# uzh-rpg/RVT

Hardware: AMD Instinct MI355X
Metric: event-tensors/sec (fwd+bwd) RVT-Base T=21 1Mpx; % MFMA roofline (higher is better)
Workload: dtype bf16; 1 GPU; RVT-Base, 1Mpx 20x360x640 (padded 384x640), T=21, B=24/GPU; global_batch=24, seq_len=21, parallelism=dp1, optimizer=AdamW(fused), hipgraph=off, upstream_grads=random cotangents on stage 2-4 features of all T frames

## Files before the change

### rvt_amd/csrc/capi_scan.hip

```cpp
#include "host.hpp"
#include "gemm.hpp"
#include "lstm_scan.hpp"
#include "lstm_scan2.hpp"
#include "lstm_scan3.hpp"

using namespace rvt;

extern "C" {
int rvt_lstm_scan_supported(int dtype, int C) {
    if (dtype != RVT_BF16 && dtype != RVT_F32) return 0;
    return C == 32 || C == 64 || C == 128;
}
}
template <class K> static int scan_grid(K kernel, int threads, int M, int tm) {
    const int resident_override = tuning().gemm_resident;
    const int n_tiles = (M + tm - 1) / tm;
    const int per_cu = resident_per_cu(kernel, threads, 1);
    return imax(1, imin(n_tiles, resident_override > 0 ? resident_override : 256 * per_cu));
}
template <class T, int C, int NW, int RB, bool W_LDS, bool W_REG = false>
static void launch_lstm_scan_fwd(const void* x_all, void* Hall, const float* c0, float* c_last, void* Csave, const void* W,
                                 const float* bias, void* gates_out, int M, int Tn, hipStream_t st) {
    constexpr int TM = (NW / (C / 32)) * RB * 32;
    auto k = lstm_scan_fwd_kernel<T, C, NW, RB, W_LDS, W_REG>;
// ... 89 lines not shown
            auto k = lstm_scan2_bwd_kernel;
            const int grid = scan_grid(k, 512, M, Scan2BwdSmem::TM);
            hipLaunchKernelGGL(k, dim3(grid), dim3(512), 0, st, (const bf16*)x_all, (const bf16*)Hall, (const bf16*)Csave, c0,
                               (const bf16*)dH, dc_last, (const bf16*)w, bias, (bf16*)dx_all, (bf16*)dh0, dc0, ws, M, T_steps);
            const size_t wn = (size_t)4 * C * 2 * C;
            FoldJobs fj;
            fj.add((const float*)ws, dw, grid, Scan2BwdSmem::REC, wn);
            fj.add((const float*)(ws + wn), db, grid, Scan2BwdSmem::REC, (size_t)4 * C);
            launch_fold_jobs(fj, st);
        }
        else if (C == 64) RVT_SCAN_BWD(bf16, 64, 4, true, false);
        else RVT_SCAN_BWD(bf16, 128, 4, false, false);
    } else {
        if (C == 32) RVT_SCAN_BWD(float, 32, 4, false, false);
        else if (C == 64) RVT_SCAN_BWD(float, 64, 4, false, false);
        else RVT_SCAN_BWD(float, 128, 4, false, false);
    }
#undef RVT_SCAN_BWD
    return check_launch("lstm_scan_bwd");
}


int rvt_lstm_scan3_rb(int C) { return (C == 256 ? tuning().lstm_scan3_rb256 : tuning().lstm_scan3_rb128) == 2 ? 2 : 1; }
int rvt_lstm_scan3_supported(int dtype, int C) {
    return dtype == RVT_BF16 && ((C == 256 && (tuning().lstm_scan3 & 1)) || (C == 128 && (tuning().lstm_scan3 & 2)));
}
int rvt_lstm_scan3_rows(int C, int M, int rb) {
    const int tm = 32 * (rb == 2 ? 2 : 1);
    return (M + tm - 1) / tm * tm;
}
int rvt_lstm_scan3_pack(const void* w, void* wp_fwd, void* wtp_bwd, int C, void* stream) {
    RVT_CHECK(C % 64 == 0 && w != nullptr, "lstm_scan3_pack: C=%d must be a multiple of 64", C);
    hipStream_t st = (hipStream_t)stream;
    const int pieces = (C / 64) * (2 * C / 16) * 8 * 64;
    const int grid = imax(1, imin(1024, (pieces + 255) / 256));
    if (wp_fwd != nullptr) hipLaunchKernelGGL(lstm_scan3_pack_kernel<false>, dim3(grid), dim3(256), 0, st, (const bf16*)w, (bf16*)wp_fwd, C);
    if (wtp_bwd != nullptr) hipLaunchKernelGGL(lstm_scan3_pack_kernel<true>, dim3(grid), dim3(256), 0, st, (const bf16*)w, (bf16*)wtp_bwd, C);
    return check_launch("lstm_scan3_pack");
}
int rvt_lstm_scan3_fwd(const void* x_all, void* Hall, const float* c0, float* c_last, void* Csave, const void* wp, const float* bias,
                       void* gsave, int dtype, int M, int C, int T_steps, int rb, void* stream) {
    RVT_CHECK(rvt_lstm_scan3_supported(dtype, C) && (rb == 1 || rb == 2), "lstm_scan3_fwd: not built for dtype=%d C=%d rb=%d", dtype, C, rb);
    RVT_CHECK(M >= 1 && T_steps >= 1 && (Csave == nullptr) == (gsave == nullptr), "lstm_scan3_fwd: empty problem, or only one of Csave / gsave");
    hipStream_t st = (hipStream_t)stream;
#define RVT_SCAN3_FWD(CC, RBB) do { auto k = lstm_scan3_fwd_kernel<CC, RBB>;                                                     \
        hipLaunchKernelGGL(k, dim3(scan_grid(k, CC, M, 32 * RBB)), dim3(CC), 0, st, (const bf16*)x_all, (bf16*)Hall, c0, c_last, \
                           (bf16*)Csave, (const bf16*)wp, bias, (bf16*)gsave, M, T_steps); } while (0)
    if (C == 256) { if (rb == 2) RVT_SCAN3_FWD(256, 2); else RVT_SCAN3_FWD(256, 1); }
    else { if (rb == 2) RVT_SCAN3_FWD(128, 2); else RVT_SCAN3_FWD(128, 1); }
#undef RVT_SCAN3_FWD
    return check_launch("lstm_scan3_fwd");
}
int rvt_lstm_scan3_bwd(const void* gsave, const void* Csave, const float* c0, const void* dH, const float* dc_last, const void* wtp,
                       void* dx_all, void* dz_all, void* dh0, float* dc0, int dtype, int M, int C, int T_steps, int rb, void* stream) {
    RVT_CHECK(rvt_lstm_scan3_supported(dtype, C) && (rb == 1 || rb == 2), "lstm_scan3_bwd: not built for dtype=%d C=%d rb=%d", dtype, C, rb);
    RVT_CHECK(M >= 1 && T_steps >= 1 && gsave != nullptr && Csave != nullptr && dx_all != nullptr && dz_all != nullptr,
              "lstm_scan3_bwd: empty problem / missing buffers");
    hipStream_t st = (hipStream_t)stream;
#define RVT_SCAN3_BWD(CC) do { auto k = lstm_scan3_bwd_kernel<CC>;                                                                       \
        hipLaunchKernelGGL(k, dim3(scan_grid(k, CC, M, 32)), dim3(CC), 0, st, (const bf16*)gsave, (const bf16*)Csave, c0, (const bf16*)dH, \
                           dc_last, (const bf16*)wtp, (bf16*)dx_all, (bf16*)dz_all, (bf16*)dh0, dc0, M, T_steps, rb); } while (0)
    if (C == 256) RVT_SCAN3_BWD(256); else RVT_SCAN3_BWD(128);
#undef RVT_SCAN3_BWD
    return check_launch("lstm_scan3_bwd");
}

}
```

### rvt_amd/csrc/capi_stage.hip

```cpp
#include <vector>
#include "host.hpp"

using namespace rvt;

namespace rvt {
int stage_blocks_fwd(const RvtStageDesc& d, const RvtStageRoutes& r, const void* inp, void* prepack, void* y0, void* x0,
                     const RvtBlockSaved* blk, int T, int B, void* stream) {
    const int C = d.C, F = T * B, dt = d.dtype;
    const int H = conv_out(d.H_in, d.k, d.stride, d.pad), W = conv_out(d.W_in, d.k, d.stride, d.pad), M = F * H * W;
    if (d.inp_u8 && rvt_stem_supported(dt, 1, d.Cin, C, d.k, d.stride, d.pad, d.w_raw)) {
        RVT_TRY(rvt_stem_fwd(inp, d.conv_w, d.ln_w, d.ln_b, y0, x0, dt, F, d.Cin, d.cin_pad, d.h_raw, d.w_raw, d.H_in, d.W_in, d.eps, stream));
    } else {
        if (d.inp_u8) {
            RVT_CHECK(prepack != nullptr, "stage forward: uint8 planes need the stem kernels (the host prepacks otherwise)");
            RVT_TRY(rvt_prepack_input(inp, 1, prepack, dt, F, d.Cin, d.h_raw, d.w_raw, d.H_in, d.W_in, d.cin_pad, stream));
            inp = prepack;
        }
        RVT_TRY(rvt_conv_fwd(inp, d.conv_w, y0, dt, F, d.H_in, d.W_in, d.cin_pad, C, d.k, d.stride, d.pad, stream));
        RVT_TRY(rvt_layernorm_fwd(y0, d.ln_w, d.ln_b, x0, dt, M, C, d.eps, stream));
    }
    const void* x = x0;
    for (int bi = 0; bi < 2 * d.num_blocks; bi++) {
        const RvtBlockWeights& bw = d.blocks[bi];
        const RvtBlockSaved& b = blk[bi];
// ... 54 lines not shown
}
}

extern "C" {

int rvt_stage_routes(const RvtStageDesc* dp, int T, int B, int save, int has_dws, int has_token_mask, RvtStageRoutes* out) {
    RVT_CHECK(dp != nullptr && out != nullptr && dp->struct_bytes == (int)sizeof(RvtStageDesc) && T >= 1 && B >= 1,
              "stage_routes: bad arguments (struct_bytes must be sizeof(RvtStageDesc) = %d)", (int)sizeof(RvtStageDesc));
    const RvtStageDesc& d = *dp;
    const RvtTuning& tn = tuning();
    const int dt = d.dtype, C = d.C, n_tok = d.ph * d.pw;
    const int Ms = B * conv_out(d.H_in, d.k, d.stride, d.pad) * conv_out(d.W_in, d.k, d.stride, d.pad);
    RvtStageRoutes r;
    memset(&r, 0, sizeof(r));

    r.attn_block = !(save && n_tok > 64) && tn.route_attn_block != 0 && rvt_attn_block_supported(dt, C, d.dim_head, n_tok);
    r.ln_linear = !r.attn_block && rvt_ln_linear_supported(dt, C, 3 * C);
    r.dgrad_ln_qkv = rvt_linear_dgrad_ln_supported(dt, C, 3 * C) != 0;
    r.dgrad_ln_fc1 = rvt_linear_dgrad_ln_supported(dt, C, 4 * C) != 0;
    r.attn_preln = (r.attn_block || r.dgrad_ln_qkv) && tn.route_attn_preln != 0 && !has_token_mask && d.num_blocks > 0 &&
                   d.blocks != nullptr && d.blocks[0].n1_w == nullptr;

    const int mlp_mode = tn.route_fused_mlp;
    const bool mlp_fused = mlp_mode != 0 && rvt_mlp_fused_supported(dt, C);
    if (mlp_mode != 0 && tn.route_mlp_bwd_fused != 0 && rvt_mlp_bwd_fused_supported(dt, C)) r.mlp_route = 1;
    else if (mlp_fused && (mlp_mode == 1 || C == 64 || C == 128)) r.mlp_route = save ? 2 : 1;
    r.mlp_bwd_both = r.mlp_route == 1 && rvt_mlp_bwd_both_supported(dt, C);
    r.mlp_bwd_dgrad = r.mlp_route == 2 && (mlp_mode == 1 || C == 64);
    r.mlp_store_pre = r.mlp_route == 2 && tn.route_mlp_store_pre != 0 && !r.mlp_bwd_dgrad;

    const int scan_mode = tn.route_lstm_scan;
    if (!has_dws && rvt_lstm_scan3_supported(dt, C) && !(C == 128 && Ms < 16384 && scan_mode != 0) && (save || T > 1)) {
        r.lstm_route = 3;
        r.lstm_scan3_rb = rvt_lstm_scan3_rb(C);
    } else if (!has_dws && scan_mode != 0 && rvt_lstm_scan_supported(dt, C) && !(scan_mode == -1 && T == 1 && !save) &&
               (scan_mode == 1 || C <= 64 || rvt_lstm_scan_saves_gates(dt, C))) {
        r.lstm_route = rvt_lstm_scan_saves_gates(dt, C) ? 2 : 1;
    }
    r.lstm_scan_wgrad = r.lstm_route == 1 && tn.route_lstm_scan_wgrad != 0 && rvt_lstm_scan_bwd_ws_floats(dt, C, Ms) > 0;
    r.conv_dgrad4 = tn.route_conv_dgrad4 != 0 && rvt_conv_dgrad4_supported(dt, d.H_in, d.W_in, d.Cin, C, d.k, d.stride, d.pad, T * B);
    r.driver_covers = !has_dws && !has_token_mask && (!save || r.mlp_route != 2);
    *out = r;
    return 0;
}

size_t rvt_stage_seq_fwd_ws_bytes(const RvtStageDesc* d, int T, int B) {
    RvtStageRoutes r;
    if (rvt_stage_routes(d, T, B, 0, 0, 0, &r) != 0) return 0;
    return stage_ws_bytes(*d, r, T, B);
}

int rvt_stage_seq_fwd(const RvtStageDesc* dp, const void* inp, const void* h0, const float* c0, void* Hall, float* c_last,
                      void* ws, size_t ws_bytes, int T, int B, void* stream) {
    RvtStageRoutes r;
    RVT_TRY(rvt_stage_routes(dp, T, B, 0, 0, 0, &r));
    const RvtStageDesc& d = *dp;
    RVT_CHECK(d.num_blocks >= 0 && d.blocks != nullptr && inp != nullptr && Hall != nullptr && c_last != nullptr, "stage_seq_fwd: bad arguments");
    RVT_CHECK((h0 == nullptr) == (c0 == nullptr), "stage_seq_fwd: h0 and c0 go together");
    RVT_CHECK(ws != nullptr && ws_bytes >= stage_ws_bytes(d, r, T, B), "stage_seq_fwd: workspace of %zu bytes < rvt_stage_seq_fwd_ws_bytes = %zu",
              ws_bytes, stage_ws_bytes(d, r, T, B));
    const int C = d.C, F = T * B, dt = d.dtype;
    const int H = conv_out(d.H_in, d.k, d.stride, d.pad), W = conv_out(d.W_in, d.k, d.stride, d.pad);
    RVT_CHECK(H % d.ph == 0 && W % d.pw == 0, "stage_seq_fwd: %dx%d not divisible by the partition %dx%d", H, W, d.ph, d.pw);
    const size_t e = elt_bytes(dt), tok = (size_t)F * H * W, act = tok * C * e;
    RVT_CHECK(tok * 4 * C < ((size_t)1 << 31), "stage_seq_fwd: %zu token rows exceed the operators' 32-bit sizes", tok);
    Carver cv{(char*)ws, ws_bytes, 256};
    void* bufs[3] = {cv.take(act), cv.take(act), cv.take(act)};
// ... 53 lines not shown
```

### rvt_amd/csrc/lstm_scan3.hpp

```cpp
#pragma once
#include "common.hpp"
#include "mlp.hpp"
#include "ppgemm.hpp"

namespace rvt {

template <int C, int RB> struct Scan3Geom {
    static constexpr int NW = C / 64, NT = 64 * NW, TM = 32 * RB;
    static constexpr int KT = C / 64;
    static constexpr int TILE = KT * TM * 128;
    static constexpr int NKF = 2 * C / 16;
    static constexpr int NKB = 4 * C / 16;
    static constexpr int PD = RB == 1 ? 4 : 8;
    static constexpr int WGS = RB == 1 ? 512 / C : 1;
    static_assert(C % 64 == 0 && NKF % PD == 0 && NKB % PD == 0, "geometry");
};

__device__ __forceinline__ bf16x8 scan3_as_frag(const u32x4& v) { return __builtin_bit_cast(bf16x8, v); }

template <int C, int RB> __device__ __forceinline__ void scan3_dma_tile(char* smem, int tile_off, const bf16* src, int rows, int wave, int lane) {
    typedef Scan3Geom<C, RB> G;
    const pp_rsrc rs = pp_make_rsrc(src, src != nullptr ? (unsigned)(rows * C * 2) : 0u);
    constexpr int NI = G::KT * (G::TM / 8), PER = NI / G::NW;
    static_assert(NI % G::NW == 0, "DMA pieces per wave");
#pragma unroll
    for (int q = 0; q < PER; q++) {
        const int u = wave * PER + q;
        const int kt = u / (G::TM / 8), rg = u % (G::TM / 8);
        const int r = 8 * rg + (lane >> 3);
        const int c = (lane & 7) ^ ((r >> 1) & 7) ^ ((r >> 4) & 7);
        pp_glds16(rs, smem, tile_off + kt * G::TM * 128 + rg * 1024, r * C * 2 + kt * 128 + c * 16, 0);
    }
}

template <int C, int RB>
__global__ void __launch_bounds__(C, (Scan3Geom<C, RB>::WGS * C) / 256)
lstm_scan3_fwd_kernel(const bf16* __restrict__ x_all, bf16* __restrict__ Hall, const float* __restrict__ c0, float* __restrict__ c_last,
                      bf16* __restrict__ Csave, const bf16* __restrict__ Wp, const float* __restrict__ bias, bf16* __restrict__ gsave,
                      int M, int Tn) {
    typedef bf16 T;
    typedef Scan3Geom<C, RB> G;
    constexpr int NW = G::NW, NT = G::NT, TM = G::TM, TILE = G::TILE, NKF = G::NKF, PD = G::PD;
    __shared__ __attribute__((aligned(1024))) char smem[4 * TILE];
    constexpr int OFF_X = 0, OFF_H = 2 * TILE;

    const int tid = threadIdx.x, lane = tid & 63, wave = wave_uniform(tid >> 6);
    const int li = lane & 31, half = lane >> 5;
    const size_t MC = (size_t)M * C;
    int ch[2];
    float nbf[2], nbi[2], nbo[2], tbg[2];
    int off0[RB][2];
#pragma unroll
    for (int cb = 0; cb < 2; cb++) {
        ch[cb] = 64 * wave + 32 * cb + li;
        nbf[cb] = bias[ch[cb]] * -1.4426950408889634f;
        nbi[cb] = bias[C + ch[cb]] * -1.4426950408889634f;
        nbo[cb] = bias[2 * C + ch[cb]] * -1.4426950408889634f;
        tbg[cb] = bias[3 * C + ch[cb]] * 2.8853900817779268f;
#pragma unroll
        for (int i = 0; i < RB; i++)
            off0[i][cb] = (int)(reinterpret_cast<char*>(opm_elem_ptr<T>(smem, TM, i * 32 + 4 * half, ch[cb])) - smem);
    }
    const pp_rsrc rw = pp_make_rsrc(Wp + (size_t)wave * NKF * 8 * 512, (unsigned)(NKF * 8 * 1024));
    const int lane16 = lane * 16;
    u32x4 bq[PD][4];
    auto issue = [&](u32x4 (&slot)[4], int p) {
#pragma unroll
        for (int j = 0; j < 4; j++) slot[j] = pp_load16(rw, ((p * 4 + j) << 10) + lane16);
    };
#pragma unroll
    for (int j = 0; j < PD; j++) issue(bq[j], j);

    const int n_tiles = (M + TM - 1) / TM;
    const size_t ntb = (size_t)n_tiles * RB;
    for (int tile = blockIdx.x; tile < n_tiles; tile += gridDim.x) {
        const int m0 = tile * TM;
        const int rows = M - m0 < TM ? M - m0 : TM;
        float creg[RB][2][16];
        lds_barrier();
        scan3_dma_tile<C, RB>(smem, OFF_H, Hall + (size_t)m0 * C, rows, wave, lane);
        scan3_dma_tile<C, RB>(smem, OFF_X, x_all + (size_t)m0 * C, rows, wave, lane);
#pragma unroll
        for (int i = 0; i < RB; i++)
#pragma unroll
            for (int cb = 0; cb < 2; cb++)
#pragma unroll
                for (int r = 0; r < 16; r++) {
                    const int row = m0 + i * 32 + acc_row(r, lane);
                    creg[i][cb][r] = (c0 != nullptr && row < M) ? c0[(size_t)row * C + ch[cb]] : 0.f;
                }
        pp_wait_vm<0>();
        lds_barrier();
        for (int t = 0; t < Tn; t++) {
            const int cur = t & 1;
            const char* const Ax = smem + OFF_X + cur * TILE;
            const char* const Ah = smem + OFF_H + cur * TILE;
            char* const An = smem + OFF_H + (cur ^ 1) * TILE;
            if (t + 1 < Tn) scan3_dma_tile<C, RB>(smem, OFF_X + (cur ^ 1) * TILE, x_all + (size_t)(t + 1) * MC + (size_t)m0 * C, rows, wave, lane);
#pragma unroll
            for (int cb = 0; cb < 2; cb++) {
                f32x16 acc[RB][4];
#pragma unroll
                for (int i = 0; i < RB; i++)
#pragma unroll
                    for (int g = 0; g < 4; g++) acc_zero(acc[i][g]);
#pragma unroll 1
                for (int k0 = 0; k0 < NKF; k0 += PD) {
#pragma unroll
                    for (int j = 0; j < PD; j++) {
                        const int ks = k0 + j;
                        const char* const A = ks < C / 16 ? Ax : Ah;
                        const int fcg = ((ks & (C / 16 - 1)) << 1) + half;
                        frag_t<T> a[RB];
#pragma unroll
                        for (int i = 0; i < RB; i++) a[i] = opm_load_frag<T>(A, TM, i * 32 + li, fcg);
#pragma unroll
                        for (int g = 0; g < 4; g++)
#pragma unroll
                            for (int i = 0; i < RB; i++) mma32(acc[i][g], a[i], scan3_as_frag(bq[j][g]));
                        int pn = cb * NKF + ks + PD;
                        if (pn >= 2 * NKF) pn -= 2 * NKF;
                        issue(bq[j], pn);
                    }
                }
#pragma unroll
                for (int i = 0; i < RB; i++) {
                    const size_t blk = (((size_t)t * ntb + (size_t)tile * RB + i) * NW + wave) * 2 + cb;
#pragma unroll
                    for (int h8 = 0; h8 < 2; h8++) {
                        float f8[8], i8[8], o8[8], g8[8], c8[8];
#pragma unroll
                        for (int e = 0; e < 8; e++) {
                            const int r = 8 * h8 + e;
                            const float f = sigmoid_zb(acc[i][0][r], nbf[cb]);
                            const float ig = sigmoid_zb(acc[i][1][r], nbi[cb]);
                            const float o = sigmoid_zb(acc[i][2][r], nbo[cb]);
                            const float g = tanh_zb(acc[i][3][r], tbg[cb]);
                            const float cn = f * creg[i][cb][r] + ig * g;
                            creg[i][cb][r] = cn;
                            *reinterpret_cast<T*>(An + acc_elem_off(off0[i][cb], r)) = (T)(o * tanh_f(cn));
                            f8[e] = f; i8[e] = ig; o8[e] = o; g8[e] = g; c8[e] = cn;
                        }
                        if (gsave != nullptr) {
                            T* const gd = gsave + (blk * 8 + h8) * 512 + lane * 8;
                            frag_store<T>(gd, frag_from_float<T>(f8));
                            frag_store<T>(gd + 2 * 512, frag_from_float<T>(i8));
                            frag_store<T>(gd + 4 * 512, frag_from_float<T>(o8));
                            frag_store<T>(gd + 6 * 512, frag_from_float<T>(g8));
                            frag_store<T>(Csave + (blk * 2 + h8) * 512 + lane * 8, frag_from_float<T>(c8));
                        }
                    }
                }
            }
            lds_barrier();
            {
                T* const hdst = Hall + (size_t)(t + 1) * MC + (size_t)m0 * C;
                constexpr int GP = C / 8;
#pragma unroll
                for (int q = 0; q < TM * GP / NT; q++) {
                    const int f = tid + q * NT;
                    const int row = f / GP, cg = f % GP;
                    if (row < rows) frag_store<T>(hdst + (size_t)row * C + cg * 8, opm_load_frag<T>(An, TM, row, cg));
                }
            }
        }
#pragma unroll
        for (int i = 0; i < RB; i++)
#pragma unroll
            for (int cb = 0; cb < 2; cb++)
#pragma unroll
                for (int r = 0; r < 16; r++) {
                    const int row = m0 + i * 32 + acc_row(r, lane);
                    if (row < M) c_last[(size_t)row * C + ch[cb]] = creg[i][cb][r];
                }
    }
}

template <int C>
__global__ void __launch_bounds__(C)
lstm_scan3_bwd_kernel(const bf16* __restrict__ gsave, const bf16* __restrict__ Csave, const float* __restrict__ c0,
                      const bf16* __restrict__ dH, const float* __restrict__ dc_last, const bf16* __restrict__ Wtp,
                      bf16* __restrict__ dx_all, bf16* __restrict__ dz_all, bf16* __restrict__ dh0, float* __restrict__ dc0,
                      int M, int Tn, int rb_fwd) {
    typedef bf16 T;
    typedef Scan3Geom<C, 1> G;
    constexpr int NW = G::NW, NT = G::NT, TM = G::TM, TILE = G::TILE, NKB = G::NKB, PD = 8;
    constexpr int DZ = 4 * TILE;
    __shared__ __attribute__((aligned(1024))) char smem[DZ + 3 * TILE];
    constexpr int OFF_DZ = 0, OFF_D = DZ, OFF_SX = DZ + 2 * TILE;
    char* const Adz = smem + OFF_DZ;
    char* const Sx = smem + OFF_SX;

    const int tid = threadIdx.x, lane = tid & 63, wave = wave_uniform(tid >> 6);
    const int li = lane & 31, half = lane >> 5;
    const size_t MC = (size_t)M * C;
    int ch[2], off0[2];
#pragma unroll
    for (int cb = 0; cb < 2; cb++) {
        ch[cb] = 64 * wave + 32 * cb + li;
        off0[cb] = (int)(reinterpret_cast<char*>(opm_elem_ptr<T>(smem, TM, 4 * half, ch[cb])) - smem);
    }
    auto dz_off = [&](int cb, int g, int r) -> int { return g * TILE + acc_elem_off(off0[cb], r); };
    const pp_rsrc rw = pp_make_rsrc(Wtp + (size_t)wave * NKB * 4 * 512, (unsigned)(NKB * 4 * 1024));
    const int lane16 = lane * 16;
    u32x4 bq[PD][4];
    auto issue = [&](u32x4 (&slot)[4], int ks) {
#pragma unroll
        for (int j = 0; j < 4; j++) slot[j] = pp_load16(rw, ((ks * 4 + j) << 10) + lane16);
    };
#pragma unroll
    for (int j = 0; j < PD; j++) issue(bq[j], j);

    const int n_tiles = (M + TM - 1) / TM;
    const size_t ntb = (size_t)((M + 32 * rb_fwd - 1) / (32 * rb_fwd)) * rb_fwd;
    for (int tile = blockIdx.x; tile < n_tiles; tile += gridDim.x) {
        const int m0 = tile * TM;
        const int rows = M - m0 < TM ? M - m0 : TM;
        float dh_rec[2][16], dc_rec[2][16];
#pragma unroll
        for (int cb = 0; cb < 2; cb++)
#pragma unroll
            for (int r = 0; r < 16; r++) {
                const int row = m0 + acc_row(r, lane);
                dh_rec[cb][r] = 0.f;
                dc_rec[cb][r] = (dc_last != nullptr && row < M) ? dc_last[(size_t)row * C + ch[cb]] : 0.f;
            }
        lds_barrier();
        scan3_dma_tile<C, 1>(smem, OFF_D + ((Tn - 1) & 1) * TILE, dH != nullptr ? dH + (size_t)(Tn - 1) * MC + (size_t)m0 * C : nullptr,
                             rows, wave, lane);
        pp_wait_vm<0>();
        lds_barrier();
        for (int t = Tn - 1; t >= 0; t--) {
            const char* const Sd = smem + OFF_D + (t & 1) * TILE;
            if (t > 0) scan3_dma_tile<C, 1>(smem, OFF_D + ((t - 1) & 1) * TILE, dH != nullptr ? dH + (size_t)(t - 1) * MC + (size_t)m0 * C : nullptr,
                                            rows, wave, lane);
#pragma unroll
            for (int cb = 0; cb < 2; cb++) {
                const size_t blk = (((size_t)t * ntb + tile) * NW + wave) * 2 + cb;
                const size_t blkp = (((size_t)(t > 0 ? t - 1 : 0) * ntb + tile) * NW + wave) * 2 + cb;
#pragma unroll
                for (int h8 = 0; h8 < 2; h8++) {
                    float f8[8], i8[8], o8[8], g8[8], cp8[8];
                    const T* const gs = gsave + (blk * 8 + h8) * 512 + lane * 8;
                    frag_to_float<T>(frag_load<T>(gs), f8);
                    frag_to_float<T>(frag_load<T>(gs + 2 * 512), i8);
                    frag_to_float<T>(frag_load<T>(gs + 4 * 512), o8);
                    frag_to_float<T>(frag_load<T>(gs + 6 * 512), g8);
                    if (t > 0) {
                        frag_to_float<T>(frag_load<T>(Csave + (blkp * 2 + h8) * 512 + lane * 8), cp8);
                    } else {
#pragma unroll
                        for (int e = 0; e < 8; e++) {
                            const int row = m0 + acc_row(8 * h8 + e, lane);
                            cp8[e] = (c0 != nullptr && row < M) ? (float)(T)c0[(size_t)row * C + ch[cb]] : 0.f;
                        }
                    }
#pragma unroll
                    for (int e = 0; e < 8; e++) {
                        const int r = 8 * h8 + e;
                        const float f = f8[e], ig = i8[e], o = o8[e], g = g8[e], cp = cp8[e];
                        const float dh = (float)*reinterpret_cast<const T*>(Sd + acc_elem_off(off0[cb], r)) + dh_rec[cb][r];
                        const float tc = tanh_f(f * cp + ig * g);
                        const float dc = dc_rec[cb][r] + dh * o * (1.f - tc * tc);
                        *reinterpret_cast<T*>(Adz + dz_off(cb, 0, r)) = (T)(dc * cp * f * (1.f - f));
                        *reinterpret_cast<T*>(Adz + dz_off(cb, 1, r)) = (T)(dc * g * ig * (1.f - ig));
                        *reinterpret_cast<T*>(Adz + dz_off(cb, 2, r)) = (T)(dh * tc * o * (1.f - o));
                        *reinterpret_cast<T*>(Adz + dz_off(cb, 3, r)) = (T)(dc * ig * (1.f - g * g));
                        dc_rec[cb][r] = dc * f;
                    }
                }
            }
            lds_barrier();
            {
                T* const zdst = dz_all + (size_t)t * MC * 4 + (size_t)m0 * 4 * C;
                constexpr int GP = 4 * C / 8;
#pragma unroll
                for (int q = 0; q < TM * GP / NT; q++) {
                    const int f = tid + q * NT;
                    const int row = f / GP, cg = f % GP;
                    if (row < rows) frag_store<T>(zdst + (size_t)row * 4 * C + cg * 8, opm_load_frag<T>(Adz, TM, row, cg));
                }
            }
            f32x16 acc2[2][2];
#pragma unroll
            for (int cb = 0; cb < 2; cb++) { acc_zero(acc2[cb][0]); acc_zero(acc2[cb][1]); }
#pragma unroll 1
            for (int k0 = 0; k0 < NKB; k0 += PD) {
#pragma unroll
                for (int j = 0; j < PD; j++) {
                    const int ks = k0 + j;
                    const frag_t<T> a = opm_load_frag<T>(Adz, TM, li, 2 * ks + half);
#pragma unroll
                    for (int cb = 0; cb < 2; cb++)
#pragma unroll
                        for (int part = 0; part < 2; part++) mma32(acc2[cb][part], a, scan3_as_frag(bq[j][cb * 2 + part]));
                    int kn = ks + PD;
                    if (kn >= NKB) kn -= NKB;
                    issue(bq[j], kn);
                }
            }
#pragma unroll
            for (int cb = 0; cb < 2; cb++)
#pragma unroll
                for (int r = 0; r < 16; r++) {
                    *reinterpret_cast<T*>(Sx + acc_elem_off(off0[cb], r)) = (T)acc2[cb][0][r];
                    dh_rec[cb][r] = acc2[cb][1][r];
                }
            lds_barrier();
            {
                T* const xdst = dx_all + (size_t)t * MC + (size_t)m0 * C;
                constexpr int GP = C / 8;
#pragma unroll
                for (int q = 0; q < TM * GP / NT; q++) {
                    const int f = tid + q * NT;
                    const int row = f / GP, cg = f % GP;
                    if (row < rows) frag_store<T>(xdst + (size_t)row * C + cg * 8, opm_load_frag<T>(Sx, TM, row, cg));
                }
            }
        }
#pragma unroll
        for (int cb = 0; cb < 2; cb++)
#pragma unroll
            for (int r = 0; r < 16; r++) {
                const int row = m0 + acc_row(r, lane);
                if (row < M) {
                    dh0[(size_t)row * C + ch[cb]] = (T)dh_rec[cb][r];
                    dc0[(size_t)row * C + ch[cb]] = dc_rec[cb][r];
                }
            }
    }
}

template <bool BWD>
__global__ void __launch_bounds__(256)
lstm_scan3_pack_kernel(const bf16* __restrict__ W, bf16* __restrict__ out, int C) {
    const int nk = BWD ? 4 * C / 16 : 2 * C / 16, per = BWD ? 4 : 8;
    const size_t total = (size_t)(C / 64) * nk * per * 64;
    for (size_t p = (size_t)blockIdx.x * 256 + threadIdx.x; p < total; p += (size_t)gridDim.x * 256) {
        const int lane = (int)(p & 63);
        size_t q = p >> 6;
        const int li = lane & 31, half = lane >> 5;
        bf16x8 v;
        if (!BWD) {
            const int g = (int)(q & 3); q >>= 2;
            const int ks = (int)(q % nk); q /= nk;
            const int cb = (int)(q & 1), w = (int)(q >> 1);
            v = *reinterpret_cast<const bf16x8*>(W + (size_t)(g * C + 64 * w + 32 * cb + li) * 2 * C + 16 * ks + 8 * half);
        } else {
            const int j = (int)(q % per); q /= per;
            const int ks = (int)(q % nk);
            const int w = (int)(q / nk);
            const int cb = j >> 1, part = j & 1;
            const int col = part * C + 64 * w + 32 * cb + li;
#pragma unroll
            for (int e = 0; e < 8; e++) v[e] = W[(size_t)(16 * ks + 8 * half + e) * 2 * C + col];
        }
        *reinterpret_cast<bf16x8*>(out + p * 8) = v;
    }
}

}
```

Before: 7488 event-tensors/s.

## Split LSTM scan3 work across twice as many waves, one 32-channel block each

The scan3 LSTM forward and backward kernels now run with 2*C threads, so each wave owns a single 32-channel block instead of two. This halves the per-wave register state and serial MMA chain, and lets weight prefetch depth and the repacked weight layout change to match. The backward kernel gains a row-block template parameter, and the default routing now picks two row blocks for large problems. The tradeoff is more waves competing for LDS and barriers, possibly lower occupancy per CU, and more per-wave A-fragment LDS traffic.

```diff
diff --git a/rvt_amd/csrc/capi_scan.hip b/rvt_amd/csrc/capi_scan.hip
--- a/rvt_amd/csrc/capi_scan.hip
+++ b/rvt_amd/csrc/capi_scan.hip
@@ -145,7 +145,7 @@
 int rvt_lstm_scan3_pack(const void* w, void* wp_fwd, void* wtp_bwd, int C, void* stream) {
     RVT_CHECK(C % 64 == 0 && w != nullptr, "lstm_scan3_pack: C=%d must be a multiple of 64", C);
     hipStream_t st = (hipStream_t)stream;
-    const int pieces = (C / 64) * (2 * C / 16) * 8 * 64;
+    const int pieces = (C / 32) * (2 * C / 16) * 4 * 64;
     const int grid = imax(1, imin(1024, (pieces + 255) / 256));
     if (wp_fwd != nullptr) hipLaunchKernelGGL(lstm_scan3_pack_kernel<false>, dim3(grid), dim3(256), 0, st, (const bf16*)w, (bf16*)wp_fwd, C);
     if (wtp_bwd != nullptr) hipLaunchKernelGGL(lstm_scan3_pack_kernel<true>, dim3(grid), dim3(256), 0, st, (const bf16*)w, (bf16*)wtp_bwd, C);
@@ -157,7 +157,7 @@
     RVT_CHECK(M >= 1 && T_steps >= 1 && (Csave == nullptr) == (gsave == nullptr), "lstm_scan3_fwd: empty problem, or only one of Csave / gsave");
     hipStream_t st = (hipStream_t)stream;
 #define RVT_SCAN3_FWD(CC, RBB) do { auto k = lstm_scan3_fwd_kernel<CC, RBB>;                                                     \
-        hipLaunchKernelGGL(k, dim3(scan_grid(k, CC, M, 32 * RBB)), dim3(CC), 0, st, (const bf16*)x_all, (bf16*)Hall, c0, c_last, \
+        hipLaunchKernelGGL(k, dim3(scan_grid(k, 2 * CC, M, 32 * RBB)), dim3(2 * CC), 0, st, (const bf16*)x_all, (bf16*)Hall, c0, c_last, \
                            (bf16*)Csave, (const bf16*)wp, bias, (bf16*)gsave, M, T_steps); } while (0)
     if (C == 256) { if (rb == 2) RVT_SCAN3_FWD(256, 2); else RVT_SCAN3_FWD(256, 1); }
     else { if (rb == 2) RVT_SCAN3_FWD(128, 2); else RVT_SCAN3_FWD(128, 1); }
@@ -170,10 +170,10 @@
     RVT_CHECK(M >= 1 && T_steps >= 1 && gsave != nullptr && Csave != nullptr && dx_all != nullptr && dz_all != nullptr,
               "lstm_scan3_bwd: empty problem / missing buffers");
     hipStream_t st = (hipStream_t)stream;
-#define RVT_SCAN3_BWD(CC) do { auto k = lstm_scan3_bwd_kernel<CC>;                                                                       \
-        hipLaunchKernelGGL(k, dim3(scan_grid(k, CC, M, 32)), dim3(CC), 0, st, (const bf16*)gsave, (const bf16*)Csave, c0, (const bf16*)dH, \
-                           dc_last, (const bf16*)wtp, (bf16*)dx_all, (bf16*)dz_all, (bf16*)dh0, dc0, M, T_steps, rb); } while (0)
-    if (C == 256) RVT_SCAN3_BWD(256); else RVT_SCAN3_BWD(128);
+#define RVT_SCAN3_BWD(CC, RBB) do { auto k = lstm_scan3_bwd_kernel<CC, RBB>;                                                             \
+        hipLaunchKernelGGL(k, dim3(scan_grid(k, 2 * CC, M, 32 * RBB)), dim3(2 * CC), 0, st, (const bf16*)gsave, (const bf16*)Csave, c0,    \
+                           (const bf16*)dH, dc_last, (const bf16*)wtp, (bf16*)dx_all, (bf16*)dz_all, (bf16*)dh0, dc0, M, T_steps, rb); } while (0)
+    if (C == 256) RVT_SCAN3_BWD(256, 1); else RVT_SCAN3_BWD(128, 1);
 #undef RVT_SCAN3_BWD
     return check_launch("lstm_scan3_bwd");
 }
diff --git a/rvt_amd/csrc/capi_stage.hip b/rvt_amd/csrc/capi_stage.hip
--- a/rvt_amd/csrc/capi_stage.hip
+++ b/rvt_amd/csrc/capi_stage.hip
@@ -110,7 +110,7 @@
     const int scan_mode = tn.route_lstm_scan;
     if (!has_dws && rvt_lstm_scan3_supported(dt, C) && !(C == 128 && Ms < 16384 && scan_mode != 0) && (save || T > 1)) {
         r.lstm_route = 3;
-        r.lstm_scan3_rb = rvt_lstm_scan3_rb(C);
+        r.lstm_scan3_rb = rvt_lstm_scan3_rb(C) == 2 || (long long)Ms * C >= (1ll << 22) ? 2 : 1;
     } else if (!has_dws && scan_mode != 0 && rvt_lstm_scan_supported(dt, C) && !(scan_mode == -1 && T == 1 && !save) &&
                (scan_mode == 1 || C <= 64 || rvt_lstm_scan_saves_gates(dt, C))) {
         r.lstm_route = rvt_lstm_scan_saves_gates(dt, C) ? 2 : 1;
diff --git a/rvt_amd/csrc/lstm_scan3.hpp b/rvt_amd/csrc/lstm_scan3.hpp
--- a/rvt_amd/csrc/lstm_scan3.hpp
+++ b/rvt_amd/csrc/lstm_scan3.hpp
@@ -6,16 +6,17 @@
 namespace rvt {
 
 template <int C, int RB> struct Scan3Geom {
-    static constexpr int NW = C / 64, NT = 64 * NW, TM = 32 * RB;
+    static constexpr int NW = C / 32, NT = 64 * NW, TM = 32 * RB;
     static constexpr int KT = C / 64;
     static constexpr int TILE = KT * TM * 128;
     static constexpr int NKF = 2 * C / 16;
     static constexpr int NKB = 4 * C / 16;
-    static constexpr int PD = RB == 1 ? 4 : 8;
-    static constexpr int WGS = RB == 1 ? 512 / C : 1;
-    static_assert(C % 64 == 0 && NKF % PD == 0 && NKB % PD == 0, "geometry");
+    static constexpr int PD = RB == 1 ? 8 : 4;
+    static constexpr int PDB = RB == 2 ? 16 : 8;
+    static constexpr int ND = RB == 2 ? 4 : 0;
+    static constexpr int WPE = 2;
+    static_assert(C % 64 == 0 && NKF % PD == 0 && NKF > PD && NKB % PDB == 0 && ND <= PD && ND <= 2 * RB, "geometry");
 };
-
 __device__ __forceinline__ bf16x8 scan3_as_frag(const u32x4& v) { return __builtin_bit_cast(bf16x8, v); }
 
 template <int C, int RB> __device__ __forceinline__ void scan3_dma_tile(char* smem, int tile_off, const bf16* src, int rows, int wave, int lane) {
@@ -34,7 +35,7 @@
 }
 
 template <int C, int RB>
-__global__ void __launch_bounds__(C, (Scan3Geom<C, RB>::WGS * C) / 256)
+__global__ void __launch_bounds__(2 * C, (Scan3Geom<C, RB>::WPE))
 lstm_scan3_fwd_kernel(const bf16* __restrict__ x_all, bf16* __restrict__ Hall, const float* __restrict__ c0, float* __restrict__ c_last,
                       bf16* __restrict__ Csave, const bf16* __restrict__ Wp, const float* __restrict__ bias, bf16* __restrict__ gsave,
                       int M, int Tn) {
@@ -45,50 +46,37 @@
     constexpr int OFF_X = 0, OFF_H = 2 * TILE;
 
     const int tid = threadIdx.x, lane = tid & 63, wave = wave_uniform(tid >> 6);
-    const int li = lane & 31, half = lane >> 5;
     const size_t MC = (size_t)M * C;
-    int ch[2];
-    float nbf[2], nbi[2], nbo[2], tbg[2];
-    int off0[RB][2];
-#pragma unroll
-    for (int cb = 0; cb < 2; cb++) {
-        ch[cb] = 64 * wave + 32 * cb + li;
-        nbf[cb] = bias[ch[cb]] * -1.4426950408889634f;
-        nbi[cb] = bias[C + ch[cb]] * -1.4426950408889634f;
-        nbo[cb] = bias[2 * C + ch[cb]] * -1.4426950408889634f;
-        tbg[cb] = bias[3 * C + ch[cb]] * 2.8853900817779268f;
-#pragma unroll
-        for (int i = 0; i < RB; i++)
-            off0[i][cb] = (int)(reinterpret_cast<char*>(opm_elem_ptr<T>(smem, TM, i * 32 + 4 * half, ch[cb])) - smem);
-    }
-    const pp_rsrc rw = pp_make_rsrc(Wp + (size_t)wave * NKF * 8 * 512, (unsigned)(NKF * 8 * 1024));
-    const int lane16 = lane * 16;
+    const int ch = 32 * wave + (lane & 31);
+    const float nbf = bias[ch] * -1.4426950408889634f;
+    const float nbi = bias[C + ch] * -1.4426950408889634f;
+    const float nbo = bias[2 * C + ch] * -1.4426950408889634f;
+    const float tbg = bias[3 * C + ch] * 2.8853900817779268f;
+    const pp_rsrc rw = pp_make_rsrc(Wp + (size_t)wave * NKF * 4 * 512, (unsigned)(NKF * 4 * 1024));
     u32x4 bq[PD][4];
-    auto issue = [&](u32x4 (&slot)[4], int p) {
+    auto issue = [&](u32x4 (&slot)[4], int p, int lane16) {
 #pragma unroll
         for (int j = 0; j < 4; j++) slot[j] = pp_load16(rw, ((p * 4 + j) << 10) + lane16);
     };
 #pragma unroll
-    for (int j = 0; j < PD; j++) issue(bq[j], j);
+    for (int j = 0; j < PD; j++) issue(bq[j], j, lane * 16);
 
     const int n_tiles = (M + TM - 1) / TM;
     const size_t ntb = (size_t)n_tiles * RB;
     for (int tile = blockIdx.x; tile < n_tiles; tile += gridDim.x) {
         const int m0 = tile * TM;
         const int rows = M - m0 < TM ? M - m0 : TM;
-        float creg[RB][2][16];
+        float creg[RB][16];
         lds_barrier();
         scan3_dma_tile<C, RB>(smem, OFF_H, Hall + (size_t)m0 * C, rows, wave, lane);
         scan3_dma_tile<C, RB>(smem, OFF_X, x_all + (size_t)m0 * C, rows, wave, lane);
 #pragma unroll
         for (int i = 0; i < RB; i++)
 #pragma unroll
-            for (int cb = 0; cb < 2; cb++)
-#pragma unroll
-                for (int r = 0; r < 16; r++) {
-                    const int row = m0 + i * 32 + acc_row(r, lane);
-                    creg[i][cb][r] = (c0 != nullptr && row < M) ? c0[(size_t)row * C + ch[cb]] : 0.f;
-                }
+            for (int r = 0; r < 16; r++) {
+                const int row = m0 + i * 32 + acc_row(r, lane);
+                creg[i][r] = (c0 != nullptr && row < M) ? c0[(size_t)row * C + ch] : 0.f;
+            }
         pp_wait_vm<0>();
         lds_barrier();
         for (int t = 0; t < Tn; t++) {
@@ -97,94 +85,107 @@
             const char* const Ah = smem + OFF_H + cur * TILE;
             char* const An = smem + OFF_H + (cur ^ 1) * TILE;
             if (t + 1 < Tn) scan3_dma_tile<C, RB>(smem, OFF_X + (cur ^ 1) * TILE, x_all + (size_t)(t + 1) * MC + (size_t)m0 * C, rows, wave, lane);
-#pragma unroll
-            for (int cb = 0; cb < 2; cb++) {
-                f32x16 acc[RB][4];
-#pragma unroll
-                for (int i = 0; i < RB; i++)
-#pragma unroll
-                    for (int g = 0; g < 4; g++) acc_zero(acc[i][g]);
+            int lk = lane;
+            opaque_vgpr(lk);
+            const int lik = lk & 31, halfk = lk >> 5, lane16 = lk * 16;
+            f32x16 acc[RB][4];
+#pragma unroll
+            for (int i = 0; i < RB; i++)
+#pragma unroll
+                for (int g = 0; g < 4; g++) acc_zero(acc[i][g]);
+            auto ksteps = [&](int k0, int nd) __attribute__((always_inline)) {
+#pragma unroll
+                for (int j = 0; j < PD; j++) {
+                    const int ks = k0 + j;
+                    const char* const A = ks < C / 16 ? Ax : Ah;
+                    const int fcg = ((ks & (C / 16 - 1)) << 1) + halfk;
+                    frag_t<T> a[RB];
+#pragma unroll
+                    for (int i = 0; i < RB; i++) a[i] = opm_load_frag<T>(A, TM, i * 32 + lik, fcg);
+#pragma unroll
+                    for (int g = 0; g < 4; g++)
+#pragma unroll
+                        for (int i = 0; i < RB; i++) mma32(acc[i][g], a[i], scan3_as_frag(bq[j][g]));
+                    if (j < PD - nd) {
+                        int pn = ks + PD;
+                        if (pn >= NKF) pn -= NKF;
+                        issue(bq[j], pn, lane16);
+                    }
+                }
+            };
 #pragma unroll 1
-                for (int k0 = 0; k0 < NKF; k0 += PD) {
-#pragma unroll
-                    for (int j = 0; j < PD; j++) {
-                        const int ks = k0 + j;
-                        const char* const A = ks < C / 16 ? Ax : Ah;
-                        const int fcg = ((ks & (C / 16 - 1)) << 1) + half;
-                        frag_t<T> a[RB];
-#pragma unroll
-                        for (int i = 0; i < RB; i++) a[i] = opm_load_frag<T>(A, TM, i * 32 + li, fcg);
-#pragma unroll
-                        for (int g = 0; g < 4; g++)
-#pragma unroll
-                            for (int i = 0; i < RB; i++) mma32(acc[i][g], a[i], scan3_as_frag(bq[j][g]));
-                        int pn = cb * NKF + ks + PD;
-                        if (pn >= 2 * NKF) pn -= 2 * NKF;
-                        issue(bq[j], pn);
-                    }
-                }
-#pragma unroll
-                for (int i = 0; i < RB; i++) {
-                    const size_t blk = (((size_t)t * ntb + (size_t)tile * RB + i) * NW + wave) * 2 + cb;
-#pragma unroll
-                    for (int h8 = 0; h8 < 2; h8++) {
-                        float f8[8], i8[8], o8[8], g8[8], c8[8];
-#pragma unroll
-                        for (int e = 0; e < 8; e++) {
-                            const int r = 8 * h8 + e;
-                            const float f = sigmoid_zb(acc[i][0][r], nbf[cb]);
-                            const float ig = sigmoid_zb(acc[i][1][r], nbi[cb]);
-                            const float o = sigmoid_zb(acc[i][2][r], nbo[cb]);
-                            const float g = tanh_zb(acc[i][3][r], tbg[cb]);
-                            const float cn = f * creg[i][cb][r] + ig * g;
-                            creg[i][cb][r] = cn;
-                            *reinterpret_cast<T*>(An + acc_elem_off(off0[i][cb], r)) = (T)(o * tanh_f(cn));
-                            f8[e] = f; i8[e] = ig; o8[e] = o; g8[e] = g; c8[e] = cn;
-                        }
-                        if (gsave != nullptr) {
-                            T* const gd = gsave + (blk * 8 + h8) * 512 + lane * 8;
-                            frag_store<T>(gd, frag_from_float<T>(f8));
-                            frag_store<T>(gd + 2 * 512, frag_from_float<T>(i8));
-                            frag_store<T>(gd + 4 * 512, frag_from_float<T>(o8));
-                            frag_store<T>(gd + 6 * 512, frag_from_float<T>(g8));
-                            frag_store<T>(Csave + (blk * 2 + h8) * 512 + lane * 8, frag_from_float<T>(c8));
-                        }
-                    }
+            for (int k0 = 0; k0 < NKF - PD; k0 += PD) ksteps(k0, 0);
+            ksteps(NKF - PD, G::ND);
+            int lg = lane;
+            opaque_vgpr(lg);
+            int off0[RB];
+#pragma unroll
+            for (int i = 0; i < RB; i++)
+                off0[i] = (int)(reinterpret_cast<char*>(opm_elem_ptr<T>(smem, TM, i * 32 + 4 * (lg >> 5), 32 * wave + (lg & 31))) - smem);
+#pragma unroll
+            for (int i = 0; i < RB; i++) {
+                const size_t blk = ((size_t)t * ntb + (size_t)tile * RB + i) * NW + wave;
+#pragma unroll
+                for (int h8 = 0; h8 < 2; h8++) {
+                    float f8[8], i8[8], o8[8], g8[8], c8[8];
+#pragma unroll
+                    for (int e = 0; e < 8; e++) {
+                        const int r = 8 * h8 + e;
+                        const float f = sigmoid_zb(acc[i][0][r], nbf);
+                        const float ig = sigmoid_zb(acc[i][1][r], nbi);
+                        const float o = sigmoid_zb(acc[i][2][r], nbo);
+                        const float g = tanh_zb(acc[i][3][r], tbg);
+                        const float cn = f * creg[i][r] + ig * g;
+                        creg[i][r] = cn;
+                        *reinterpret_cast<T*>(An + acc_elem_off(off0[i], r)) = (T)(o * tanh_f(cn));
+                        f8[e] = f; i8[e] = ig; o8[e] = o; g8[e] = g; c8[e] = cn;
+                    }
+                    if (gsave != nullptr) {
+                        T* const gd = gsave + (blk * 8 + h8) * 512 + lg * 8;
+                        frag_store<T>(gd, frag_from_float<T>(f8));
+                        frag_store<T>(gd + 2 * 512, frag_from_float<T>(i8));
+                        frag_store<T>(gd + 4 * 512, frag_from_float<T>(o8));
+                        frag_store<T>(gd + 6 * 512, frag_from_float<T>(g8));
+                        frag_store<T>(Csave + (blk * 2 + h8) * 512 + lg * 8, frag_from_float<T>(c8));
+                    }
+                    if (2 * i + h8 < G::ND) issue(bq[PD - G::ND + 2 * i + h8], PD - G::ND + 2 * i + h8, lg * 16);
                 }
             }
             lds_barrier();
             {
                 T* const hdst = Hall + (size_t)(t + 1) * MC + (size_t)m0 * C;
                 constexpr int GP = C / 8;
+                int tq = tid;
+                opaque_vgpr(tq);
 #pragma unroll
                 for (int q = 0; q < TM * GP / NT; q++) {
-                    const int f = tid + q * NT;
+                    const int f = tq + q * NT;
                     const int row = f / GP, cg = f % GP;
                     if (row < rows) frag_store<T>(hdst + (size_t)row * C + cg * 8, opm_load_frag<T>(An, TM, row, cg));
                 }
             }
         }
+        int le = lane;
+        opaque_vgpr(le);
 #pragma unroll
         for (int i = 0; i < RB; i++)
 #pragma unroll
-            for (int cb = 0; cb < 2; cb++)
-#pragma unroll
-                for (int r = 0; r < 16; r++) {
-                    const int row = m0 + i * 32 + acc_row(r, lane);
-                    if (row < M) c_last[(size_t)row * C + ch[cb]] = creg[i][cb][r];
-                }
+            for (int r = 0; r < 16; r++) {
+                const int row = m0 + i * 32 + acc_row(r, le);
+                if (row < M) c_last[(size_t)row * C + 32 * wave + (le & 31)] = creg[i][r];
+            }
     }
 }
 
-template <int C>
-__global__ void __launch_bounds__(C)
+template <int C, int RBB>
+__global__ void __launch_bounds__(2 * C, RBB == 1 ? 2 : 1)
 lstm_scan3_bwd_kernel(const bf16* __restrict__ gsave, const bf16* __restrict__ Csave, const float* __restrict__ c0,
                       const bf16* __restrict__ dH, const float* __restrict__ dc_last, const bf16* __restrict__ Wtp,
                       bf16* __restrict__ dx_all, bf16* __restrict__ dz_all, bf16* __restrict__ dh0, float* __restrict__ dc0,
                       int M, int Tn, int rb_fwd) {
     typedef bf16 T;
-    typedef Scan3Geom<C, 1> G;
-    constexpr int NW = G::NW, NT = G::NT, TM = G::TM, TILE = G::TILE, NKB = G::NKB, PD = 8;
+    typedef Scan3Geom<C, RBB> G;
+    constexpr int NW = G::NW, NT = G::NT, TM = G::TM, TILE = G::TILE, NKB = G::NKB, PD = G::PDB;
     constexpr int DZ = 4 * TILE;
     __shared__ __attribute__((aligned(1024))) char smem[DZ + 3 * TILE];
     constexpr int OFF_DZ = 0, OFF_D = DZ, OFF_SX = DZ + 2 * TILE;
@@ -192,81 +193,86 @@
     char* const Sx = smem + OFF_SX;
 
     const int tid = threadIdx.x, lane = tid & 63, wave = wave_uniform(tid >> 6);
-    const int li = lane & 31, half = lane >> 5;
     const size_t MC = (size_t)M * C;
-    int ch[2], off0[2];
-#pragma unroll
-    for (int cb = 0; cb < 2; cb++) {
-        ch[cb] = 64 * wave + 32 * cb + li;
-        off0[cb] = (int)(reinterpret_cast<char*>(opm_elem_ptr<T>(smem, TM, 4 * half, ch[cb])) - smem);
-    }
-    auto dz_off = [&](int cb, int g, int r) -> int { return g * TILE + acc_elem_off(off0[cb], r); };
-    const pp_rsrc rw = pp_make_rsrc(Wtp + (size_t)wave * NKB * 4 * 512, (unsigned)(NKB * 4 * 1024));
-    const int lane16 = lane * 16;
-    u32x4 bq[PD][4];
-    auto issue = [&](u32x4 (&slot)[4], int ks) {
-#pragma unroll
-        for (int j = 0; j < 4; j++) slot[j] = pp_load16(rw, ((ks * 4 + j) << 10) + lane16);
+    const int ch = 32 * wave + (lane & 31);
+    auto elem0 = [&](int i, int l) -> int { return (int)(reinterpret_cast<char*>(opm_elem_ptr<T>(smem, TM, i * 32 + 4 * (l >> 5), 32 * wave + (l & 31))) - smem); };
+    const pp_rsrc rw = pp_make_rsrc(Wtp + (size_t)wave * NKB * 2 * 512, (unsigned)(NKB * 2 * 1024));
+    u32x4 bq[PD][2];
+    auto issue = [&](u32x4 (&slot)[2], int ks, int lane16) {
+#pragma unroll
+        for (int j = 0; j < 2; j++) slot[j] = pp_load16(rw, ((ks * 2 + j) << 10) + lane16);
     };
 #pragma unroll
-    for (int j = 0; j < PD; j++) issue(bq[j], j);
+    for (int j = 0; j < PD; j++) issue(bq[j], j, lane * 16);
 
     const int n_tiles = (M + TM - 1) / TM;
     const size_t ntb = (size_t)((M + 32 * rb_fwd - 1) / (32 * rb_fwd)) * rb_fwd;
     for (int tile = blockIdx.x; tile < n_tiles; tile += gridDim.x) {
         const int m0 = tile * TM;
         const int rows = M - m0 < TM ? M - m0 : TM;
-        float dh_rec[2][16], dc_rec[2][16];
-#pragma unroll
-        for (int cb = 0; cb < 2; cb++)
+        float dh_rec[RBB][16], dc_rec[RBB][16];
+#pragma unroll
+        for (int i = 0; i < RBB; i++)
 #pragma unroll
             for (int r = 0; r < 16; r++) {
-                const int row = m0 + acc_row(r, lane);
-                dh_rec[cb][r] = 0.f;
-                dc_rec[cb][r] = (dc_last != nullptr && row < M) ? dc_last[(size_t)row * C + ch[cb]] : 0.f;
+                const int row = m0 + i * 32 + acc_row(r, lane);
+                dh_rec[i][r] = 0.f;
+                dc_rec[i][r] = (dc_last != nullptr && row < M) ? dc_last[(size_t)row * C + ch] : 0.f;
             }
         lds_barrier();
-        scan3_dma_tile<C, 1>(smem, OFF_D + ((Tn - 1) & 1) * TILE, dH != nullptr ? dH + (size_t)(Tn - 1) * MC + (size_t)m0 * C : nullptr,
-                             rows, wave, lane);
+        scan3_dma_tile<C, RBB>(smem, OFF_D + ((Tn - 1) & 1) * TILE, dH != nullptr ? dH + (size_t)(Tn - 1) * MC + (size_t)m0 * C : nullptr,
+                               rows, wave, lane);
         pp_wait_vm<0>();
         lds_barrier();
         for (int t = Tn - 1; t >= 0; t--) {
             const char* const Sd = smem + OFF_D + (t & 1) * TILE;
-            if (t > 0) scan3_dma_tile<C, 1>(smem, OFF_D + ((t - 1) & 1) * TILE, dH != nullptr ? dH + (size_t)(t - 1) * MC + (size_t)m0 * C : nullptr,
-                                            rows, wave, lane);
-#pragma unroll
-            for (int cb = 0; cb < 2; cb++) {
-                const size_t blk = (((size_t)t * ntb + tile) * NW + wave) * 2 + cb;
-                const size_t blkp = (((size_t)(t > 0 ? t - 1 : 0) * ntb + tile) * NW + wave) * 2 + cb;
+            if (t > 0) scan3_dma_tile<C, RBB>(smem, OFF_D + ((t - 1) & 1) * TILE, dH != nullptr ? dH + (size_t)(t - 1) * MC + (size_t)m0 * C : nullptr,
+                                              rows, wave, lane);
+            int lg = lane;
+            opaque_vgpr(lg);
+            int off0[RBB];
+#pragma unroll
+            for (int i = 0; i < RBB; i++) off0[i] = elem0(i, lg);
+            auto dz_off = [&](int i, int g, int r) -> int { return g * TILE + acc_elem_off(off0[i], r); };
+#pragma unroll
+            for (int i = 0; i < RBB; i++) {
+                const bool live = i == 0 || 32 * i < rows;
+                const size_t blk = ((size_t)t * ntb + (size_t)tile * RBB + i) * NW + wave;
+                const size_t blkp = ((size_t)(t > 0 ? t - 1 : 0) * ntb + (size_t)tile * RBB + i) * NW + wave;
 #pragma unroll
                 for (int h8 = 0; h8 < 2; h8++) {
                     float f8[8], i8[8], o8[8], g8[8], cp8[8];
-                    const T* const gs = gsave + (blk * 8 + h8) * 512 + lane * 8;
-                    frag_to_float<T>(frag_load<T>(gs), f8);
-                    frag_to_float<T>(frag_load<T>(gs + 2 * 512), i8);
-                    frag_to_float<T>(frag_load<T>(gs + 4 * 512), o8);
-                    frag_to_float<T>(frag_load<T>(gs + 6 * 512), g8);
-                    if (t > 0) {
-                        frag_to_float<T>(frag_load<T>(Csave + (blkp * 2 + h8) * 512 + lane * 8), cp8);
+                    if (live) {
+                        const T* const gs = gsave + (blk * 8 + h8) * 512 + lg * 8;
+                        frag_to_float<T>(frag_load<T>(gs), f8);
+                        frag_to_float<T>(frag_load<T>(gs + 2 * 512), i8);
+                        frag_to_float<T>(frag_load<T>(gs + 4 * 512), o8);
+                        frag_to_float<T>(frag_load<T>(gs + 6 * 512), g8);
                     } else {
 #pragma unroll
+                        for (int e = 0; e < 8; e++) f8[e] = i8[e] = o8[e] = g8[e] = 0.f;
+                    }
+                    if (t > 0 && live) {
+                        frag_to_float<T>(frag_load<T>(Csave + (blkp * 2 + h8) * 512 + lg * 8), cp8);
+                    } else {
+#pragma unroll
                         for (int e = 0; e < 8; e++) {
-                            const int row = m0 + acc_row(8 * h8 + e, lane);
-                            cp8[e] = (c0 != nullptr && row < M) ? (float)(T)c0[(size_t)row * C + ch[cb]] : 0.f;
+                            const int row = m0 + i * 32 + acc_row(8 * h8 + e, lane);
+                            cp8[e] = (c0 != nullptr && row < M) ? (float)(T)c0[(size_t)row * C + ch] : 0.f;
                         }
                     }
 #pragma unroll
                     for (int e = 0; e < 8; e++) {
                         const int r = 8 * h8 + e;
                         const float f = f8[e], ig = i8[e], o = o8[e], g = g8[e], cp = cp8[e];
-                        const float dh = (float)*reinterpret_cast<const T*>(Sd + acc_elem_off(off0[cb], r)) + dh_rec[cb][r];
+                        const float dh = (float)*reinterpret_cast<const T*>(Sd + acc_elem_off(off0[i], r)) + dh_rec[i][r];
                         const float tc = tanh_f(f * cp + ig * g);
-                        const float dc = dc_rec[cb][r] + dh * o * (1.f - tc * tc);
-                        *reinterpret_cast<T*>(Adz + dz_off(cb, 0, r)) = (T)(dc * cp * f * (1.f - f));
-                        *reinterpret_cast<T*>(Adz + dz_off(cb, 1, r)) = (T)(dc * g * ig * (1.f - ig));
-                        *reinterpret_cast<T*>(Adz + dz_off(cb, 2, r)) = (T)(dh * tc * o * (1.f - o));
-                        *reinterpret_cast<T*>(Adz + dz_off(cb, 3, r)) = (T)(dc * ig * (1.f - g * g));
-                        dc_rec[cb][r] = dc * f;
+                        const float dc = dc_rec[i][r] + dh * o * (1.f - tc * tc);
+                        *reinterpret_cast<T*>(Adz + dz_off(i, 0, r)) = (T)(dc * cp * f * (1.f - f));
+                        *reinterpret_cast<T*>(Adz + dz_off(i, 1, r)) = (T)(dc * g * ig * (1.f - ig));
+                        *reinterpret_cast<T*>(Adz + dz_off(i, 2, r)) = (T)(dh * tc * o * (1.f - o));
+                        *reinterpret_cast<T*>(Adz + dz_off(i, 3, r)) = (T)(dc * ig * (1.f - g * g));
+                        dc_rec[i][r] = dc * f;
                     }
                 }
             }
@@ -274,58 +280,71 @@
             {
                 T* const zdst = dz_all + (size_t)t * MC * 4 + (size_t)m0 * 4 * C;
                 constexpr int GP = 4 * C / 8;
+                int tq = tid;
+                opaque_vgpr(tq);
 #pragma unroll
                 for (int q = 0; q < TM * GP / NT; q++) {
-                    const int f = tid + q * NT;
+                    const int f = tq + q * NT;
                     const int row = f / GP, cg = f % GP;
                     if (row < rows) frag_store<T>(zdst + (size_t)row * 4 * C + cg * 8, opm_load_frag<T>(Adz, TM, row, cg));
                 }
             }
-            f32x16 acc2[2][2];
-#pragma unroll
-            for (int cb = 0; cb < 2; cb++) { acc_zero(acc2[cb][0]); acc_zero(acc2[cb][1]); }
+            int lk = lane;
+            opaque_vgpr(lk);
+            const int lik = lk & 31, halfk = lk >> 5, lane16 = lk * 16;
+            f32x16 acc2[RBB][2];
+#pragma unroll
+            for (int i = 0; i < RBB; i++) { acc_zero(acc2[i][0]); acc_zero(acc2[i][1]); }
 #pragma unroll 1
             for (int k0 = 0; k0 < NKB; k0 += PD) {
 #pragma unroll
                 for (int j = 0; j < PD; j++) {
                     const int ks = k0 + j;
-                    const frag_t<T> a = opm_load_frag<T>(Adz, TM, li, 2 * ks + half);
-#pragma unroll
-                    for (int cb = 0; cb < 2; cb++)
-#pragma unroll
-                        for (int part = 0; part < 2; part++) mma32(acc2[cb][part], a, scan3_as_frag(bq[j][cb * 2 + part]));
+                    frag_t<T> a[RBB];
+#pragma unroll
+                    for (int i = 0; i < RBB; i++) a[i] = opm_load_frag<T>(Adz, TM, i * 32 + lik, 2 * ks + halfk);
+#pragma unroll
+                    for (int part = 0; part < 2; part++)
+#pragma unroll
+                        for (int i = 0; i < RBB; i++) mma32(acc2[i][part], a[i], scan3_as_frag(bq[j][part]));
                     int kn = ks + PD;
                     if (kn >= NKB) kn -= NKB;
-                    issue(bq[j], kn);
-                }
-            }
-#pragma unroll
-            for (int cb = 0; cb < 2; cb++)
+                    issue(bq[j], kn, lane16);
+                }
+            }
+            int lx = lane;
+            opaque_vgpr(lx);
+#pragma unroll
+            for (int i = 0; i < RBB; i++)
 #pragma unroll
                 for (int r = 0; r < 16; r++) {
-                    *reinterpret_cast<T*>(Sx + acc_elem_off(off0[cb], r)) = (T)acc2[cb][0][r];
-                    dh_rec[cb][r] = acc2[cb][1][r];
+                    *reinterpret_cast<T*>(Sx + acc_elem_off(elem0(i, lx), r)) = (T)acc2[i][0][r];
+                    dh_rec[i][r] = acc2[i][1][r];
                 }
             lds_barrier();
             {
                 T* const xdst = dx_all + (size_t)t * MC + (size_t)m0 * C;
                 constexpr int GP = C / 8;
+                int tq = tid;
+                opaque_vgpr(tq);
 #pragma unroll
                 for (int q = 0; q < TM * GP / NT; q++) {
-                    const int f = tid + q * NT;
+                    const int f = tq + q * NT;
                     const int row = f / GP, cg = f % GP;
                     if (row < rows) frag_store<T>(xdst + (size_t)row * C + cg * 8, opm_load_frag<T>(Sx, TM, row, cg));
                 }
             }
         }
-#pragma unroll
-        for (int cb = 0; cb < 2; cb++)
+        int le = lane;
+        opaque_vgpr(le);
+#pragma unroll
+        for (int i = 0; i < RBB; i++)
 #pragma unroll
             for (int r = 0; r < 16; r++) {
-                const int row = m0 + acc_row(r, lane);
+                const int row = m0 + i * 32 + acc_row(r, le);
                 if (row < M) {
-                    dh0[(size_t)row * C + ch[cb]] = (T)dh_rec[cb][r];
-                    dc0[(size_t)row * C + ch[cb]] = dc_rec[cb][r];
+                    dh0[(size_t)row * C + 32 * wave + (le & 31)] = (T)dh_rec[i][r];
+                    dc0[(size_t)row * C + 32 * wave + (le & 31)] = dc_rec[i][r];
                 }
             }
     }
@@ -334,24 +353,20 @@
 template <bool BWD>
 __global__ void __launch_bounds__(256)
 lstm_scan3_pack_kernel(const bf16* __restrict__ W, bf16* __restrict__ out, int C) {
-    const int nk = BWD ? 4 * C / 16 : 2 * C / 16, per = BWD ? 4 : 8;
-    const size_t total = (size_t)(C / 64) * nk * per * 64;
+    const int nk = BWD ? 4 * C / 16 : 2 * C / 16, per = BWD ? 2 : 4;
+    const size_t total = (size_t)(C / 32) * nk * per * 64;
     for (size_t p = (size_t)blockIdx.x * 256 + threadIdx.x; p < total; p += (size_t)gridDim.x * 256) {
         const int lane = (int)(p & 63);
         size_t q = p >> 6;
         const int li = lane & 31, half = lane >> 5;
+        const int j = (int)(q % per); q /= per;
+        const int ks = (int)(q % nk);
+        const int w = (int)(q / nk);
         bf16x8 v;
         if (!BWD) {
-            const int g = (int)(q & 3); q >>= 2;
-            const int ks = (int)(q % nk); q /= nk;
-            const int cb = (int)(q & 1), w = (int)(q >> 1);
-            v = *reinterpret_cast<const bf16x8*>(W + (size_t)(g * C + 64 * w + 32 * cb + li) * 2 * C + 16 * ks + 8 * half);
+            v = *reinterpret_cast<const bf16x8*>(W + (size_t)(j * C + 32 * w + li) * 2 * C + 16 * ks + 8 * half);
         } else {
-            const int j = (int)(q % per); q /= per;
-            const int ks = (int)(q % nk);
-            const int w = (int)(q / nk);
-            const int cb = j >> 1, part = j & 1;
-            const int col = part * C + 64 * w + 32 * cb + li;
+            const int col = j * C + 32 * w + li;
 #pragma unroll
             for (int e = 0; e < 8; e++) v[e] = W[(size_t)(16 * ks + 8 * half + e) * 2 * C + col];
         }
```

Result: faster. 7581 event-tensors/s, median of 6 (+1.2%).
